# XiangFeng-Wen/STF-Unet

Hardware: AMD Instinct MI355X
Metric: training samples/sec (256x256 DCE-MRI frames) (higher is better)
Workload: dtype bf16; 1 GPU; cfg2 UNet(in=8,base_c=64) 256x256 train step; model=UNet, global_batch=64, per_gpu_batch=64, seq_len=8, parallelism=dp1, ddp_hook=False

## Files before the change

include/stfunet.h:

```cpp
#ifndef STFUNET_H
#define STFUNET_H
#include <stddef.h>
#include <stdint.h>

#ifdef __cplusplus
extern "C" {
#endif

typedef void* stf_stream_t;

typedef struct stf_conv_geom {
  int N;
  int Hs, Ws, Cs;
  int src_cstride;
  int Hd, Wd;
  int R, S;
  int stride, pad;
  int transposed;
} stf_conv_geom;

typedef struct stf_lstm_epi {
  const float* c_prev;
  float* c_out;
  void* h_out;
// ... 58 lines not shown

int stf_channel_sum(const void* x, int x_cstride, int M, int C, float* partial,
                    float* out, stf_stream_t stream);
int stf_stat_sums(const float* stats, int tiles, int Nout, int c0, int C, float* out, stf_stream_t stream);

int stf_bn_finalize(float* stats, int tiles, int groups, int C, int64_t M,
                    const float* gamma, const float* beta, float momentum, float eps,
                    float* running_mean, float* running_var, float* mean, float* invstd,
                    float* scale, float* shift, stf_stream_t stream);
typedef struct stf_bn_run_desc {
  const float* stats;
  float* running_mean;
  float* running_var;
  int64_t Mg;
  int tiles, groups, C;
  float momentum;
} stf_bn_run_desc;
int stf_bn_running_batch(const stf_bn_run_desc* descs, int count, stf_stream_t stream);
int stf_bn_act(const void* y, int y_cstride, int N, int H, int W, int C, int groups,
               const float* scale, const float* shift, int relu, const void* res,
               int res_cstride, const float* res_scale, const float* res_shift, void* out,
               int out_cstride, void* pooled, stf_stream_t stream);
int stf_bn_bwd_tiles(int N, int H, int W, int C, int groups, int pooled);
int stf_bn_bwd_reduce(const void* dz, int dz_cstride, const void* dpool, const void* y,
                      int y_cstride, int N, int H, int W, int C, int groups,
                      const float* scale, const float* shift, const float* mean,
                      const float* invstd, int mask_mode, const void* mask_src,
                      int mask_cstride, void* g_out, float* partial, stf_stream_t stream);
int stf_bn_bwd_finalize(float* partial, int tiles, int groups, int C, int64_t M,
                        const float* gamma, const float* mean, const float* invstd,
                        float* dgamma, float* dbeta, float* coef, stf_stream_t stream);
typedef struct stf_bn_gsum_desc {
  const float* partial;
  float* dgamma;
  float* dbeta;
  int tiles, groups, C;
} stf_bn_gsum_desc;
int stf_bn_groupsum_batch(const stf_bn_gsum_desc* descs, int count, stf_stream_t stream);
int stf_bn_bwd_apply_tiles(int64_t M, int C);
int stf_bn_bwd_apply(const void* g, int g_cstride, const void* y, int y_cstride, int64_t M,
                     int C, int groups, const float* mask_scale, const float* mask_shift,
                     const float* coef, void* dy, int dy_cstride, float* bias_partial,
                     float* dbias, stf_stream_t stream);

int stf_head_fwd(const void* y, int N, int H, int W, int C, const float* scale,
                 const float* shift, const float* w, const float* bias, int classes,
                 float* logits, stf_stream_t stream);
int stf_head_bwd(const float* dlogits, const void* y, int N, int H, int W, int C,
                 const float* scale, const float* shift, const float* mean,
                 const float* invstd, const float* w, int classes, void* g_out,
                 float* bn_partial, float* head_partial, float* dw, float* db,
                 stf_stream_t stream);
int stf_head_tiles(int N, int H, int W, int C);

int stf_loss_scratch_floats(int N, int classes);
int stf_loss_fwd(const float* logits, const int64_t* target, int N, int H, int W,
                 int classes, float* terms, float* loss, stf_stream_t stream);
int stf_loss_bwd(const float* logits, const int64_t* target, int N, int H, int W,
                 int classes, const float* terms, const float* grad_out, float* dlogits,
                 stf_stream_t stream);
int stf_loss_opt_scratch_floats(int N, int classes);
int stf_loss_opt_fwd(const float* logits, const int64_t* target, int N, int H, int W, int classes,
                     const float* class_weight, int ignore_index, int dice, float* terms,
                     float* loss, stf_stream_t stream);
int stf_loss_opt_bwd(const float* logits, const int64_t* target, int N, int H, int W, int classes,
                     const float* class_weight, int ignore_index, int dice, const float* terms,
                     const float* grad_out, float* dlogits, stf_stream_t stream);

int stf_adamw(float* p, const float* g, float* m, float* v, int64_t n, float lr,
              float beta1, float beta2, float eps, float weight_decay, float bc1,
              float bc2, stf_stream_t stream);
int stf_adamw_dev(float* p, const float* g, float* m, float* v, int64_t n, const float* hyper,
                  float beta1, float beta2, float eps, float weight_decay, stf_stream_t stream);
int stf_adamw_amp(float* p, const float* g, float* m, float* v, int64_t n, float* hyper,
                  const float* grad_scale, const float* found_inf, float beta1, float beta2, float eps,
                  float weight_decay, stf_stream_t stream);

int stf_pack_input(const float* x, int N, int C, int H, int W, int Cpad, void* out,
                   stf_stream_t stream);
int stf_pack_weight(const float* w, int d0, int d1, int R, int S, int mode, int cpad,
                    void* out, stf_stream_t stream);
typedef struct stf_pack_desc {
  const float* w;
  void* out;
  int d0, d1, R, S, mode, cpad;
} stf_pack_desc;
int stf_pack_weights(const stf_pack_desc* descs, int count, int64_t max_elems, stf_stream_t stream);
int stf_pack_tiles(int d0, int d1, int R, int S, int mode, int cpad);
int stf_pack_weights_tiled(const stf_pack_desc* descs, int count, int max_tiles, stf_stream_t stream);

int stf_pack_sequence(const float* x, int B, int Ttot, int C, int H, int W, int T, int P,
                      int Cpad, void* out, stf_stream_t stream);

int stf_stem_im2col(const float* x, int B, int Ttot, int C, int H, int W, int T, int P, int KS,
                    int stride, int pad, int Kpad, void* out, stf_stream_t stream);
int stf_stem_conv7_grid(int B, int T, int H, int W);
int stf_stem_conv7(const float* x, int B, int Ttot, int H, int W, int T, const void* w, void* y, float* stats,
                   stf_stream_t stream);
int stf_stem_wgrad7(const float* x, int B, int Ttot, int H, int W, int T, const void* dy, float* ws,
                    stf_stream_t stream);
int stf_stem_dgrad7(const void* dy, const float* w, int B, int Ttot, int Cf, int H, int W, int T, float* dx,
                    stf_stream_t stream);
int stf_maxpool3s2_fwd(const void* x, int N, int H, int W, int C, void* out, void* argmax,
                       stf_stream_t stream);
int stf_maxpool3s2_bwd(const void* argmax, const void* dout, int N, int H, int W, int C, void* dx,
                       stf_stream_t stream);
// ... 109 lines not shown
```

stf-unet_amd/csrc/common.h:

```cpp
#pragma once
#include <hip/hip_runtime.h>
#include <stdint.h>

#include <tuple>
#include <type_traits>
#include <utility>

#ifdef STF_FP16
typedef _Float16 e16;
#else
typedef __bf16 e16;
#endif
typedef e16 e16x8 __attribute__((ext_vector_type(8)));
typedef e16 e16x4 __attribute__((ext_vector_type(4)));
typedef short short4v __attribute__((ext_vector_type(4)));
typedef float f32x4 __attribute__((ext_vector_type(4)));
typedef float f32x16 __attribute__((ext_vector_type(16)));
typedef unsigned int u32x4v __attribute__((ext_vector_type(4)));

#define STF_DEV __device__ __forceinline__

STF_DEV float e2f(e16 v) { return (float)v; }
STF_DEV e16 f2e(float v) { return (e16)v; }

// ... 12 lines not shown
  return __uint_as_float(w << 16);
#endif
}
STF_DEV float hi16(uint32_t w) {
#ifdef STF_FP16
  return (float)__builtin_bit_cast(_Float16, (uint16_t)(w >> 16));
#else
  return __uint_as_float(w & 0xffff0000u);
#endif
}

STF_DEV void unpack8(const uint4& u, float (&f)[8]) {
  const uint32_t w[4] = {u.x, u.y, u.z, u.w};
#pragma unroll
  for (int i = 0; i < 4; ++i) {
    f[2 * i] = lo16(w[i]);
    f[2 * i + 1] = hi16(w[i]);
  }
}

STF_DEV uint32_t pack2(float a, float b) {
  e16 x = f2e(a), y = f2e(b);
  return (uint32_t)__builtin_bit_cast(uint16_t, x) | ((uint32_t)__builtin_bit_cast(uint16_t, y) << 16);
}

STF_DEV uint4 pack8(const float (&f)[8]) {
  return make_uint4(pack2(f[0], f[1]), pack2(f[2], f[3]), pack2(f[4], f[5]), pack2(f[6], f[7]));
}

STF_DEV float round_e(float v) { return e2f(f2e(v)); }

STF_DEV float sigm(float x) { return __builtin_amdgcn_rcpf(1.f + __expf(-x)); }
STF_DEV float tanh_f(float x) { return __builtin_fmaf(2.f, sigm(2.f * x), -1.f); }

STF_DEV void lstm_cell_fwd(float pi, float pf, float pg, float po, float cp, float& gi, float& gf, float& gg,
                           float& go, float& c, float& h) {
#pragma clang fp contract(off)
  gi = sigm(pi); gf = sigm(pf); gg = tanh_f(pg); go = sigm(po);
  c = __builtin_fmaf(gf, cp, gi * gg);
  h = go * tanh_f(c);
}
STF_DEV void lstm_cell_bwd(float gi, float gf, float gg, float go, float ct, float cp, float dh, float dcn,
                           float& d_i, float& d_f, float& d_g, float& d_o, float& dcp) {
#pragma clang fp contract(off)
  const float tc = tanh_f(ct);
  const float dct = __builtin_fmaf(dh * go, __builtin_fmaf(-tc, tc, 1.f), dcn);
  d_o = ((dh * tc) * go) * (1.f - go);
  d_i = ((dct * gg) * gi) * (1.f - gi);
  d_g = (dct * gi) * __builtin_fmaf(-gg, gg, 1.f);
  d_f = ((dct * cp) * gf) * (1.f - gf);
  dcp = dct * gf;
}

STF_DEV float wave_sum(float v) {
#pragma unroll
  for (int o = 32; o > 0; o >>= 1) v += __shfl_xor(v, o, 64);
  return v;
}

template <int CTRL>
STF_DEV float dpp_f(float v) {
  return __int_as_float(__builtin_amdgcn_update_dpp(0, __float_as_int(v), CTRL, 0xF, 0xF, true));
}

STF_DEV float row16_reduce_scatter(const float (&v)[16], int r) {
  float a[8], b[4], c[2];
  const bool h3 = r & 8, h2 = r & 4, h1 = r & 2, h0 = r & 1;
#pragma unroll
  for (int k = 0; k < 8; ++k) a[k] = (h3 ? v[k + 8] : v[k]) + dpp_f<0x140>(h3 ? v[k] : v[k + 8]);
#pragma unroll
  for (int k = 0; k < 4; ++k) b[k] = (h2 ? a[k + 4] : a[k]) + dpp_f<0x141>(h2 ? a[k] : a[k + 4]);
#pragma unroll
  for (int k = 0; k < 2; ++k) c[k] = (h1 ? b[k + 2] : b[k]) + dpp_f<0x1B>(h1 ? b[k] : b[k + 2]);
  return (h0 ? c[1] : c[0]) + dpp_f<0xB1>(h0 ? c[0] : c[1]);
}

STF_DEV double wave_sum_d(double v) {
#pragma unroll
  for (int o = 32; o > 0; o >>= 1) v += __shfl_xor(v, o, 64);
  return v;
}

namespace stf {
struct PlanOp {
  virtual ~PlanOp() {}
  virtual hipError_t run() const = 0;
};
bool plan_recording();
void plan_append(PlanOp* op, hipStream_t s);

template <class... A>
struct KernelOp final : PlanOp {
  const void* fn;
  dim3 grid, block;
  unsigned shmem;
  hipStream_t stream;
  std::tuple<A...> args;
  template <class... B>
  KernelOp(const void* f, dim3 g, dim3 b, unsigned sh, hipStream_t s, B&&... a)
      : fn(f), grid(g), block(b), shmem(sh), stream(s), args(std::forward<B>(a)...) {}
  hipError_t run() const override {
    return std::apply(
        [this](const A&... a) {
          void* p[sizeof...(A) + 1] = {const_cast<void*>(static_cast<const void*>(&a))...};
          return hipLaunchKernel(fn, grid, block, p, shmem, stream);
        },
// ... 36 lines not shown
```

stf-unet_amd/csrc/loss.hip:

```cpp
#include "common.h"
#include "../../include/stfunet.h"
#include "reduce.h"

namespace {

constexpr int NT = 256;
constexpr int MAXK = 4;
constexpr int LCHUNK = 64;
constexpr float DICE_EPS = 1e-6f;

STF_DEV void load8f(const float* p, float (&v)[8]) {
  const float4 a = *reinterpret_cast<const float4*>(p);
  const float4 b = *reinterpret_cast<const float4*>(p + 4);
  v[0] = a.x; v[1] = a.y; v[2] = a.z; v[3] = a.w; v[4] = b.x; v[5] = b.y; v[6] = b.z; v[7] = b.w;
}

STF_DEV float lane_group_sum(float v, int CG) {
  if (CG >= 2) v += dpp_f<0xB1>(v);
  if (CG >= 4) v += dpp_f<0x4E>(v);
  if (CG >= 8) v += dpp_f<0x141>(v);
  if (CG >= 16) v += dpp_f<0x140>(v);
  for (int o = 16; o < CG; o <<= 1) v += __shfl_xor(v, o, 64);
  return v;
}

int head_tiles(long units) {
  long t = (units + NT - 1) / NT;
  return (int)(t < 1 ? 1 : (t > 1024 ? 1024 : t));
}

template <int K>
__global__ void head_fwd_kernel(const uint16_t* __restrict__ y, long P, int HW, int C,
                                const float* __restrict__ scale, const float* __restrict__ shift,
                                const float* __restrict__ w, const float* __restrict__ bias,
                                float* __restrict__ logits) {
  constexpr int U = 4;
  const int CG = C / 8, cgs = __builtin_ctz(CG);
  const int units = (int)(P * CG);
  const int cg = (int)((blockIdx.x * NT + threadIdx.x) & (CG - 1));
  float sc[8], sh[8], wk[K][8], bk[K];
  load8f(scale + cg * 8, sc);
  load8f(shift + cg * 8, sh);
#pragma unroll
  for (int k = 0; k < K; ++k) { load8f(w + k * C + cg * 8, wk[k]); bk[k] = bias[k]; }
  const int stride = gridDim.x * NT;
  for (int u0 = blockIdx.x * NT; u0 < units; u0 += stride * U) {
    uint4 raw[U];
#pragma unroll
    for (int r = 0; r < U; ++r) {
      const int u = u0 + r * stride + threadIdx.x;
      raw[r] = u < units ? *reinterpret_cast<const uint4*>(y + (size_t)(u >> cgs) * C + cg * 8) : make_uint4(0, 0, 0, 0);
    }
#pragma unroll
    for (int r = 0; r < U; ++r) {
      const int u = u0 + r * stride + threadIdx.x;
      float v[8], acc[K];
      unpack8(raw[r], v);
#pragma unroll
      for (int k = 0; k < K; ++k) acc[k] = 0.f;
#pragma unroll
      for (int j = 0; j < 8; ++j) {
        const float a = fmaxf(v[j] * sc[j] + sh[j], 0.f);
#pragma unroll
        for (int k = 0; k < K; ++k) acc[k] += a * wk[k][j];
      }
#pragma unroll
      for (int k = 0; k < K; ++k) acc[k] = lane_group_sum(acc[k], CG);
      if (u < units && cg == 0) {
        const int pix = u >> cgs, n = pix / HW, hw = pix - n * HW;
#pragma unroll
        for (int k = 0; k < K; ++k) logits[(size_t)(n * K + k) * HW + hw] = acc[k] + bk[k];
      }
    }
  }
}

template <int K>
__global__ void head_bwd_kernel(const float* __restrict__ dlogits, const uint16_t* __restrict__ y, long P, int HW,
                                int C, const float* __restrict__ scale, const float* __restrict__ shift,
                                const float* __restrict__ mean, const float* __restrict__ invstd,
                                const float* __restrict__ w, uint16_t* __restrict__ g_out,
                                float* __restrict__ bn_partial, float* __restrict__ head_partial) {
  constexpr int NV = 16 + 8 * K + K;
  __shared__ float red[NT][NV + 1];
  const int CG = C / 8, cgs = __builtin_ctz(CG);
  const int units = (int)(P * CG);
  const int gt = blockIdx.x * NT + threadIdx.x;
  const int cg = gt & (CG - 1);
  float sc[8], sh[8], mu[8], is[8], wk[K][8];
  load8f(scale + cg * 8, sc);
  load8f(shift + cg * 8, sh);
  load8f(mean + cg * 8, mu);
  load8f(invstd + cg * 8, is);
#pragma unroll
  for (int k = 0; k < K; ++k) load8f(w + k * C + cg * 8, wk[k]);
  float sg[8] = {0, 0, 0, 0, 0, 0, 0, 0}, sgx[8] = {0, 0, 0, 0, 0, 0, 0, 0}, dw[K][8], db[K];
#pragma unroll
  for (int k = 0; k < K; ++k) {
    db[k] = 0.f;
#pragma unroll
    for (int j = 0; j < 8; ++j) dw[k][j] = 0.f;
  }
  constexpr int U = 1;
  const int S = gridDim.x * NT;
  for (int u0 = gt; u0 < units; u0 += S * U) {
    float dlr[U][K];
    uint4 yr[U];
    int pixr[U];
#pragma unroll
    for (int r = 0; r < U; ++r) {
      const int u = u0 + r * S;
      const bool ok = u < units;
      const int pix = ok ? u >> cgs : 0, n = pix / HW, hw = pix - n * HW;
      pixr[r] = ok ? pix : -1;
#pragma unroll
      for (int k = 0; k < K; ++k) dlr[r][k] = ok ? dlogits[(size_t)(n * K + k) * HW + hw] : 0.f;
      yr[r] = ok ? *reinterpret_cast<const uint4*>(y + (size_t)pix * C + cg * 8) : make_uint4(0, 0, 0, 0);
    }
#pragma unroll
    for (int r = 0; r < U; ++r) {
    if (pixr[r] < 0) continue;
    const int pix = pixr[r];
    const float* dl = dlr[r];
    float v[8], g[8];
    unpack8(yr[r], v);
#pragma unroll
    for (int j = 0; j < 8; ++j) {
      const float z = v[j] * sc[j] + sh[j];
      const float a = fmaxf(z, 0.f);
      float da = 0.f;
#pragma unroll
      for (int k = 0; k < K; ++k) { da += dl[k] * wk[k][j]; dw[k][j] += dl[k] * a; }
      g[j] = z > 0.f ? da : 0.f;
      sg[j] += g[j];
      sgx[j] += g[j] * (v[j] - mu[j]) * is[j];
    }
    if (cg == 0) {
#pragma unroll
      for (int k = 0; k < K; ++k) db[k] += dl[k];
    }
    *reinterpret_cast<uint4*>(g_out + (size_t)pix * C + cg * 8) = pack8(g);
    }
  }
#pragma unroll
  for (int j = 0; j < 8; ++j) { red[threadIdx.x][j] = sg[j]; red[threadIdx.x][8 + j] = sgx[j]; }
#pragma unroll
  for (int k = 0; k < K; ++k) {
#pragma unroll
    for (int j = 0; j < 8; ++j) red[threadIdx.x][16 + k * 8 + j] = dw[k][j];
    red[threadIdx.x][16 + 8 * K + k] = db[k];
  }
  __syncthreads();
  for (int c = threadIdx.x; c < C; c += NT) {
    const int gg = c / 8, j = c - gg * 8;
    float a = 0.f, b = 0.f;
    for (int t = gg; t < NT; t += CG) { a += red[t][j]; b += red[t][8 + j]; }
    bn_partial[(size_t)blockIdx.x * 2 * C + c] = a;
    bn_partial[(size_t)blockIdx.x * 2 * C + C + c] = b;
  }
  const int HC = K * (C + 1);
  for (int e = threadIdx.x; e < HC; e += NT) {
    float a = 0.f;
    if (e < K * C) {
      const int k = e / C, c = e - k * C, gg = c / 8, j = c - gg * 8;
      for (int t = gg; t < NT; t += CG) a += red[t][16 + k * 8 + j];
    } else {
      const int k = e - K * C;
      for (int t = 0; t < NT; t += CG) a += red[t][16 + 8 * K + k];
    }
    head_partial[(size_t)blockIdx.x * HC + e] = a;
  }
}

template <int K>
__global__ void loss_fwd_kernel(const float* __restrict__ logits, const int64_t* __restrict__ target, int HW,
                                float* __restrict__ part) {
  constexpr int NV = 3 * K + 1;
  __shared__ float red[NT / 64][NV];
  const int n = blockIdx.y;
  float s[NV];
#pragma unroll
  for (int i = 0; i < NV; ++i) s[i] = 0.f;
  for (int hw = blockIdx.x * NT + threadIdx.x; hw < HW; hw += gridDim.x * NT) {
    float z[K], e[K], mx = -INFINITY;
#pragma unroll
    for (int k = 0; k < K; ++k) { z[k] = logits[((long)n * K + k) * HW + hw]; mx = fmaxf(mx, z[k]); }
    float se = 0.f;
#pragma unroll
    for (int k = 0; k < K; ++k) { e[k] = expf(z[k] - mx); se += e[k]; }
    const int t = (int)target[(long)n * HW + hw];
    const float inv = 1.f / se, lse = logf(se);
#pragma unroll
    for (int k = 0; k < K; ++k) {
      const float p = e[k] * inv;
      const float tk = t == k ? 1.f : 0.f;
      s[3 * k] += p * tk;
      s[3 * k + 1] += p;
      s[3 * k + 2] += tk;
      if (t == k) s[3 * K] += lse - (z[k] - mx);
    }
  }
#pragma unroll
  for (int i = 0; i < NV; ++i) s[i] = wave_sum(s[i]);
  if ((threadIdx.x & 63) == 0)
#pragma unroll
    for (int i = 0; i < NV; ++i) red[threadIdx.x >> 6][i] = s[i];
  __syncthreads();
  if (threadIdx.x < NV) {
    float a = 0.f;
    for (int wv = 0; wv < NT / 64; ++wv) a += red[wv][threadIdx.x];
    part[((size_t)n * gridDim.x + blockIdx.x) * NV + threadIdx.x] = a;
  }
}

template <int K>
__global__ void loss_finalize_kernel(const float* __restrict__ part, int N, int HW, float* __restrict__ terms,
                                     float* __restrict__ loss) {
  constexpr int NV = 3 * K + 1;
  __shared__ double acc[64][NV];
  double ce = 0.0, dsum = 0.0;
  for (int base = 0; base < N; base += 64) {
    const int n = base + (int)threadIdx.x;
    if (threadIdx.x < 64) {
// ... 195 lines not shown
      }
      G[k] = dscale * dd;
      pg += p[k] * G[k];
    }
    const float cs = wt * inv_w;
#pragma unroll
    for (int k = 0; k < K; ++k) {
      const float tk = t == k ? 1.f : 0.f;
      const float g = go * ((p[k] - tk) * cs + p[k] * (G[k] - pg));
      dlogits[(n * K + k) * HW + hw] = keep ? g : 0.f;
    }
  }
}

__global__ void sum_tiles_kernel(const float* __restrict__ partial, int tiles, int C, int split,
                                 float* __restrict__ out, float* __restrict__ out2) {
  const int c = blockIdx.x * blockDim.x + threadIdx.x;
  if (c >= C) return;
  double s = 0.0;
  for (int t = 0; t < tiles; ++t) s += partial[(size_t)t * C + c];
  if (c < split) out[c] = (float)s;
  else out2[c - split] = (float)s;
}

bool head_ok(int C) { return C % 8 == 0 && C / 8 <= 64 && 64 % (C / 8) == 0; }

}

#define STF_KDISPATCH(K_, EXPR)             \
  switch (K_) {                             \
    case 1: { constexpr int KK = 1; EXPR; } break; \
    case 2: { constexpr int KK = 2; EXPR; } break; \
    case 3: { constexpr int KK = 3; EXPR; } break; \
    case 4: { constexpr int KK = 4; EXPR; } break; \
    default: return STF_EINVAL;             \
  }

extern "C" int stf_head_tiles(int N, int H, int W, int C) { return head_tiles((long)N * H * W * (C / 8)); }

extern "C" int stf_head_fwd(const void* y, int N, int H, int W, int C, const float* scale, const float* shift,
                            const float* w, const float* bias, int classes, float* logits, stf_stream_t stream) {
  if (!head_ok(C)) return STF_EINVAL;
  const long P = (long)N * H * W, units = P * (C / 8);
  if (units >= (1L << 31)) return STF_EINVAL;
  long blocks = (units + NT - 1) / NT;
  if (blocks > 8192) blocks = 8192;
  hipStream_t s = (hipStream_t)stream;
  STF_KDISPATCH(classes, hipLaunchKernelGGL(head_fwd_kernel<KK>, dim3(blocks), dim3(NT), 0, s, (const uint16_t*)y,
                                            P, H * W, C, scale, shift, w, bias, logits));
  STF_CHECK_LAUNCH();
  return 0;
}

extern "C" int stf_head_bwd(const float* dlogits, const void* y, int N, int H, int W, int C, const float* scale,
                            const float* shift, const float* mean, const float* invstd, const float* w, int classes,
                            void* g_out, float* bn_partial, float* head_partial, float* dw, float* db,
                            stf_stream_t stream) {
  if (!head_ok(C) || (long)N * H * W * (C / 8) >= (1L << 31)) return STF_EINVAL;
  const long P = (long)N * H * W;
  const int tiles = stf_head_tiles(N, H, W, C);
  hipStream_t s = (hipStream_t)stream;
  STF_KDISPATCH(classes, hipLaunchKernelGGL(head_bwd_kernel<KK>, dim3(tiles), dim3(NT), 0, s, dlogits,
                                            (const uint16_t*)y, P, H * W, C, scale, shift, mean, invstd, w,
                                            (uint16_t*)g_out, bn_partial, head_partial));
  STF_CHECK_LAUNCH();
  const int HC = classes * (C + 1);
  const int S = stf::colsum_stage1(head_partial, tiles, HC, s);
  hipLaunchKernelGGL(sum_tiles_kernel, dim3((HC + 255) / 256), dim3(256), 0, s, head_partial, S, HC, classes * C,
                     dw, db);
  STF_CHECK_LAUNCH();
  return 0;
}

extern "C" int stf_loss_scratch_floats(int N, int classes) {
  return N * classes * 3 + 1 + N * LCHUNK * (3 * classes + 1);
}

extern "C" int stf_loss_fwd(const float* logits, const int64_t* target, int N, int H, int W, int classes,
                            float* terms, float* loss, stf_stream_t stream) {
  hipStream_t s = (hipStream_t)stream;
  float* part = terms + N * classes * 3 + 1;
  STF_KDISPATCH(classes, {
    hipLaunchKernelGGL(loss_fwd_kernel<KK>, dim3(LCHUNK, N), dim3(NT), 0, s, logits, target, H * W, part);
    hipLaunchKernelGGL(loss_finalize_kernel<KK>, dim3(1), dim3(64), 0, s, part, N, H * W, terms, loss);
  });
  STF_CHECK_LAUNCH();
  return 0;
}

extern "C" int stf_loss_bwd(const float* logits, const int64_t* target, int N, int H, int W, int classes,
                            const float* terms, const float* grad_out, float* dlogits, stf_stream_t stream) {
  hipStream_t s = (hipStream_t)stream;
  const long P = (long)N * H * W;
  long blocks = (P + NT - 1) / NT;
  if (blocks > 8192) blocks = 8192;
  STF_KDISPATCH(classes, hipLaunchKernelGGL(loss_bwd_kernel<KK>, dim3(blocks), dim3(NT), 0, s, logits, target, N,
                                            H * W, terms, grad_out, dlogits));
  STF_CHECK_LAUNCH();
  return 0;
}

extern "C" int stf_loss_opt_scratch_floats(int N, int classes) {
  return N * classes * 3 + 2 + N * LCHUNK * (3 * classes + 2);
}

static bool loss_opt_ok(int classes, int ignore_index) {
  return classes >= 1 && classes <= MAXK && !(ignore_index >= 0 && ignore_index < classes);
}

extern "C" int stf_loss_opt_fwd(const float* logits, const int64_t* target, int N, int H, int W, int classes,
                                const float* class_weight, int ignore_index, int dice, float* terms, float* loss,
                                stf_stream_t stream) {
  if (!loss_opt_ok(classes, ignore_index)) return STF_EINVAL;
  hipStream_t s = (hipStream_t)stream;
  float* part = terms + N * classes * 3 + 2;
  STF_KDISPATCH(classes, {
    hipLaunchKernelGGL(loss_opt_fwd_kernel<KK>, dim3(LCHUNK, N), dim3(NT), 0, s, logits, target, H * W, class_weight,
                       ignore_index, part);
    hipLaunchKernelGGL(loss_opt_finalize_kernel<KK>, dim3(1), dim3(64), 0, s, part, N, dice, terms, loss);
  });
  STF_CHECK_LAUNCH();
  return 0;
// ... 16 lines not shown
```

stf-unet_amd/stfunet/_lib.py:

```python
import contextlib
import ctypes
import os

import torch

_HERE = os.path.dirname(os.path.abspath(__file__))
LIB_PATH = os.path.join(_HERE, "libstfunet_hip.so")
LIB_PATH = os.environ.get("STF_LIB", LIB_PATH)
LIB_PATH_F16 = os.environ.get("STF_LIB_F16", os.path.join(os.path.dirname(LIB_PATH), "libstfunet_hip_f16.so"))
LIB_PATHS = {torch.bfloat16: LIB_PATH, torch.float16: LIB_PATH_F16}
STORAGE_CODE = {torch.bfloat16: 0, torch.float16: 1}

BUILD_INFO = os.path.join(_HERE, "build_info.json")
_SRC_DIRS = (os.path.join(_HERE, "..", "csrc"), os.path.join(_HERE, "..", "..", "include"))


def _sha(paths):
    import hashlib
    h = hashlib.sha256()
    for p in paths:
        h.update(os.path.basename(p).encode())
        with open(p, "rb") as f:
            h.update(f.read())
    return h.hexdigest()[:16]
# ... 35 lines not shown
class ConvGeom(ctypes.Structure):
    _fields_ = [(n, c_int) for n in ("N", "Hs", "Ws", "Cs", "src_cstride", "Hd", "Wd", "R", "S",
                                     "stride", "pad", "transposed")]


class LstmEpi(ctypes.Structure):
    _fields_ = [("c_prev", P), ("c_out", P), ("h_out", P), ("h_cstride", c_int), ("gates", P),
                ("backward", c_int), ("dh", P), ("dh_cstride", c_int), ("dc_next", P), ("dc_prev", P),
                ("dgates", P)]


class BnrEpi(ctypes.Structure):
    _fields_ = [("y", P), ("y_cstride", c_int), ("scale", P), ("shift", P), ("mean", P), ("invstd", P),
                ("relu", c_int), ("partial", P)]


class IgemmArgs(ctypes.Structure):
    _fields_ = [("g", ConvGeom), ("src", P), ("wgt", P), ("Nout", c_int), ("dst", P),
                ("dst_cstride", c_int), ("bias", P), ("stats", P), ("scatter2x2", c_int),
                ("group_rows", c_int), ("accumulate", c_int), ("lstm", ctypes.POINTER(LstmEpi)),
                ("bnr", ctypes.POINTER(BnrEpi)), ("ws", P)]


class WgradArgs(ctypes.Structure):
    _fields_ = [("g", ConvGeom), ("dy", P), ("dy_cstride", c_int), ("Nout", c_int), ("x", P),
                ("ws", P), ("splits", c_int), ("grid_blocks", c_int)]


_SIGS = {
    "stf_igemm_stat_tiles": (c_int, [ctypes.POINTER(IgemmArgs)]),
    "stf_igemm_ws_bytes": (c_size_t, [ctypes.POINTER(IgemmArgs)]),
    "stf_igemm_bnr_tiles": (c_int, [ctypes.POINTER(IgemmArgs)]),
    "stf_igemm_kernel_name": (ctypes.c_char_p, [ctypes.POINTER(IgemmArgs)]),
    "stf_wgrad_kernel_name": (ctypes.c_char_p, [ctypes.POINTER(WgradArgs)]),
    "stf_igemm": (c_int, [ctypes.POINTER(IgemmArgs), P]),
    "stf_wgrad_plan": (c_int, [ctypes.POINTER(WgradArgs), ctypes.POINTER(c_int), ctypes.POINTER(c_size_t)]),
    "stf_wgrad": (c_int, [ctypes.POINTER(WgradArgs), P]),
    "stf_wgrad_reduce": (c_int, [P, c_int, c_int, c_int, c_int, c_int, P, P]),
    "stf_channel_sum": (c_int, [P, c_int, c_int, c_int, P, P, P]),
    "stf_bn_finalize": (c_int, [P, c_int, c_int, c_int, c_int64, P, P, c_float, c_float, P, P, P, P, P, P, P]),
    "stf_bn_running_batch": (c_int, [P, c_int, P]),
    "stf_bn_groupsum_batch": (c_int, [P, c_int, P]),
    "stf_bn_act": (c_int, [P, c_int, c_int, c_int, c_int, c_int, c_int, P, P, c_int, P, c_int, P, P, P, c_int, P,
                           P]),
    "stf_bn_bwd_tiles": (c_int, [c_int, c_int, c_int, c_int, c_int, c_int]),
    "stf_bn_bwd_reduce": (c_int, [P, c_int, P, P, c_int, c_int, c_int, c_int, c_int, c_int, P, P, P, P, c_int, P,
                                  c_int, P, P, P]),
    "stf_bn_bwd_finalize": (c_int, [P, c_int, c_int, c_int, c_int64, P, P, P, P, P, P, P]),
    "stf_bn_bwd_apply_tiles": (c_int, [c_int64, c_int]),
    "stf_bn_bwd_apply": (c_int, [P, c_int, P, c_int, c_int64, c_int, c_int, P, P, P, P, c_int, P, P, P]),
    "stf_head_fwd": (c_int, [P, c_int, c_int, c_int, c_int, P, P, P, P, c_int, P, P]),
    "stf_head_bwd": (c_int, [P, P, c_int, c_int, c_int, c_int, P, P, P, P, P, c_int, P, P, P, P, P, P]),
    "stf_head_tiles": (c_int, [c_int, c_int, c_int, c_int]),
    "stf_loss_scratch_floats": (c_int, [c_int, c_int]),
    "stf_loss_fwd": (c_int, [P, P, c_int, c_int, c_int, c_int, P, P, P]),
    "stf_loss_bwd": (c_int, [P, P, c_int, c_int, c_int, c_int, P, P, P, P]),
    "stf_loss_opt_scratch_floats": (c_int, [c_int, c_int]),
    "stf_loss_opt_fwd": (c_int, [P, P, c_int, c_int, c_int, c_int, P, c_int, c_int, P, P, P]),
    "stf_loss_opt_bwd": (c_int, [P, P, c_int, c_int, c_int, c_int, P, c_int, c_int, P, P, P, P]),
    "stf_adamw": (c_int, [P, P, P, P, c_int64, c_float, c_float, c_float, c_float, c_float, c_float, c_float,
                          P]),
    "stf_adamw_dev": (c_int, [P, P, P, P, c_int64, P, c_float, c_float, c_float, c_float, P]),
    "stf_adamw_amp": (c_int, [P, P, P, P, c_int64, P, P, P, c_float, c_float, c_float, c_float, P]),
    "stf_pack_input": (c_int, [P, c_int, c_int, c_int, c_int, c_int, P, P]),
    "stf_pack_weight": (c_int, [P, c_int, c_int, c_int, c_int, c_int, c_int, P, P]),
    "stf_pack_weights": (c_int, [P, c_int, c_int64, P]),
    "stf_augment_frames": (c_int, [P, P, c_int, P, P, c_int, c_int, c_float, c_float, P, P]),
    "stf_augment_masks": (c_int, [P, P, c_int, P, c_int, P, P]),
    "stf_pack_tiles": (c_int, [c_int, c_int, c_int, c_int, c_int, c_int]),
    "stf_pack_weights_tiled": (c_int, [P, c_int, c_int, P]),
    "stf_pack_sequence": (c_int, [P, c_int, c_int, c_int, c_int, c_int, c_int, c_int, c_int, P, P]),
    "stf_eval_counts": (c_int, [P, P, c_int, c_int, c_int64, c_int64, P, P, P]),
    "stf_lstm_coop_sync_bytes": (c_size_t, [c_int, c_int]),
    "stf_lstm_coop_supported": (c_int, [c_int]),
    "stf_lstm_coop_fwd": (c_int, [P, P, P, c_int, c_int, c_int, P, P, c_int, P, P, c_int, c_uint, P]),
    "stf_lstm_coop_bwd": (c_int, [P, P, P, c_int, c_int, c_int, P, c_int, P, P, c_int, P, c_int, c_uint, P]),
    "stf_lstm_coop_error": (c_int, [P, c_int, c_int, P, P]),
    "stf_bilinear_ac_fwd": (c_int, [P, c_int, c_int, c_int, c_int, c_int, P, c_int, c_int, c_int, P]),
    "stf_bilinear_ac_bwd": (c_int, [P, c_int, c_int, c_int, c_int, c_int, P, c_int, c_int, c_int, P]),
    "stf_stat_sums": (c_int, [P, c_int, c_int, c_int, c_int, P, P]),
    "stf_bilinear_ac_bwd_tsum": (c_int, [P, c_int, c_int, c_int, c_int, c_int, c_int, P, c_int64, c_int64, c_int,
                                         c_int, P]),
    "stf_eval_counts_sm": (c_int, [P, P, P, c_int, c_int, c_int64, c_int64, P, P, P]),
    "stf_predict_mask": (c_int, [P, P, c_int, c_int, c_int64, c_int, c_int, c_float, c_int64, P, P, P]),
    "stf_predict_overlay_scratch_bytes": (c_size_t, [c_int, c_int64]),
    "stf_predict_overlay": (c_int, [P, c_int64, P, c_int, c_int, c_int, c_int, c_int, c_int, c_float, c_int, P, P,
                                    P]),
    "stf_tofts_forward": (c_int, [P, P, P, c_int, c_int, P, P, P, P, P, c_int, c_float, P, P]),
    "stf_tofts_fit": (c_int, [P, c_int, c_int, P, P, P, P, P, c_int, c_float, c_int, c_int, P, c_float, c_float,
                              c_float, P, P, P]),
    "stf_stem_im2col": (c_int, [P, c_int, c_int, c_int, c_int, c_int, c_int, c_int, c_int, c_int, c_int, c_int, P,
                                P]),
    "stf_stem_conv7_grid": (c_int, [c_int, c_int, c_int, c_int]),
    "stf_stem_conv7": (c_int, [P, c_int, c_int, c_int, c_int, c_int, P, P, P, P]),
    "stf_stem_wgrad7": (c_int, [P, c_int, c_int, c_int, c_int, c_int, P, P, P]),
    "stf_stem_dgrad7": (c_int, [P, P, c_int, c_int, c_int, c_int, c_int, c_int, P, P]),
    "stf_maxpool3s2_fwd": (c_int, [P, c_int, c_int, c_int, c_int, P, P, P]),
    "stf_maxpool3s2_bwd": (c_int, [P, P, c_int, c_int, c_int, c_int, P, P]),
    "stf_bn_act_maxpool3s2": (c_int, [P, c_int, c_int, c_int, c_int, c_int, P, P, P, P, P]),
    "stf_bn_bwd_reduce_pool3": (c_int, [P, P, P, c_int, c_int, c_int, c_int, c_int, P, P, P, P, P, P]),
    "stf_bn_bwd_apply_pool3": (c_int, [P, P, P, c_int, c_int, c_int, c_int, c_int, P, P, P, P, P]),
    "stf_lstm_pack": (c_int, [P, P, P, P, c_int, P, P, P, P]),
    "stf_lstm_unpack_grad": (c_int, [P, P, c_int, P, P, P, P, P]),
    "stf_lstm_seq_fwd": (c_int, [P, P, P, c_int, c_int, c_int, P, P, c_int, P]),
    "stf_lstm_seq_supported": (c_int, [c_int]),
    "stf_lstm_seq_bwd": (c_int, [P, P, P, P, c_int, c_int, c_int, P, P, c_int, P, P, c_int, P]),
# ... 108 lines not shown
```

stf-unet_amd/stfunet/unet.py:

```python

import torch
import torch.nn as nn

from . import _lib, nhwc
from .flat import FlatParams
from .nhwc import Feat, new_feat
from .plan import StepRuntime


def _double_conv(cin, cout):
    return nn.Sequential(nn.Conv2d(cin, cout, 3, padding=1), nn.BatchNorm2d(cout), nn.ReLU(inplace=True),
                         nn.Conv2d(cout, cout, 3, padding=1), nn.BatchNorm2d(cout), nn.ReLU(inplace=True))


def _cpad(c):
    return (c + 7) // 8 * 8


class _Saved:
    pass


class DoubleConvProgram:

# ... 112 lines not shown
        dev = x.device
        S = _Saved()
        src = nhwc.pack_input(x, _cpad(m.in_channels))
        S.enc, S.cats = [], []
        h, w = H, W
        for lvl in self.levels:
            C = lvl.cout
            cat = new_feat(N, h, w, 2 * C, dev)
            pooled = new_feat(N, h // 2, w // 2, C, dev)
            S.enc.append(lvl.forward(src, training, need_bwd, out=cat.slice(C, C), pooled=pooled))
            S.cats.append(cat)
            src = pooled
            h, w = h // 2, w // 2
        Cb = self.bott.cout
        a_b = new_feat(N, h, w, Cb, dev)
        S.bott = self.bott.forward(src, training, need_bwd, out=a_b)
        cur = a_b
        S.dec, S.dec_in = [], []
        for i, (up, dec) in enumerate(zip(self.ups, self.decs)):
            cat = S.cats[3 - i]
            Clo = dec.cout
            wt = nhwc.pack_weight(up.weight, 2)
            nhwc.igemm(cur, wt, 4 * Clo, cat.slice(0, Clo), 1, 1, 1, 0, bias=up.bias.detach(), scatter2x2=True)
            S.dec_in.append(cur)
            last = i == 3
            if not last:
                out = new_feat(cat.N, cat.H, cat.W, Clo, dev)
                S.dec.append(dec.forward(cat, training, need_bwd, out=out))
                cur = out
            else:
                s = dec.forward(cat, training, True)
                S.dec.append(s)
        s = S.dec[-1]
        K = m.out_conv.out_channels
        logits = nhwc.empty((N, K, H, W), torch.float32, dev)
        S.head_w = m.out_conv.weight.detach().reshape(K, -1).contiguous()
        nhwc.call("stf_head_fwd", s.y2.ptr(), N, H, W, s.y2.C, nhwc._p(s.bn2.scale), nhwc._p(s.bn2.shift),
                  nhwc._p(S.head_w), nhwc._p(m.out_conv.bias.detach()), K, nhwc._p(logits), nhwc.stream())
        if not need_bwd:
            S.enc = S.cats = S.dec = None
        nhwc.flush_batches_tracked()
        return logits, (S if need_bwd else None)

    def _backward(self, S, dlogits):
        m = self.m
        gv = self.flat.grad_view
        dev = dlogits.device
        dlogits = dlogits.contiguous().float()
        s = S.dec[-1]
        N, K, H, W = dlogits.shape
        C = s.y2.C
        lib = nhwc._lib.load()
        tiles = lib.stf_head_tiles(N, H, W, C)
        g = new_feat(N, H, W, C, dev)
        bnp = nhwc.empty(tiles * 2 * C, torch.float32, dev)
        hp = nhwc.empty((tiles + 1) * K * (C + 1), torch.float32, dev)
        nhwc.call("stf_head_bwd", nhwc._p(dlogits), s.y2.ptr(), N, H, W, C, nhwc._p(s.bn2.scale),
                  nhwc._p(s.bn2.shift), nhwc._p(s.bn2.mean), nhwc._p(s.bn2.invstd), nhwc._p(S.head_w), K,
                  g.ptr(), nhwc._p(bnp), nhwc._p(hp), nhwc._p(gv(m.out_conv.weight)),
                  nhwc._p(gv(m.out_conv.bias)), nhwc.stream())
        dec1 = self.decs[3]
        dy2 = nhwc.bn_backward_from_partial(g, s.y2, s.bn2, dec1.blk[4], bnp, tiles, gv(dec1.blk[4].weight),
                                            gv(dec1.blk[4].bias), gv(dec1.blk[3].bias))
        dcat, cst, ctiles = dec1.backward(s, self.flat, True, dy2=dy2, dsrc_stats=True)
        self._done(dec1.blk)
        dcats = [None] * 4
        dcats[0] = (dcat, cst, ctiles)
        for i in (3, 2, 1, 0):
            up = self.ups[i]
            dcat, cst, ctiles = dcats[3 - i]
            dcats[3 - i] = dcat
            Clo = self.decs[i].cout
            dup = dcat.slice(0, Clo)
            src = S.dec_in[i]
            nhwc.wgrad(src, dup, 2, 2, 2, 0, gv(up.weight))
            nhwc.stat_sums(cst, ctiles, dcat.C, 0, Clo, gv(up.bias))
            dsrc = new_feat(src.N, src.H, src.W, src.C, dev)
            nhwc.igemm(dup, nhwc.pack_weight(up.weight, 3), src.C, dsrc, 2, 2, 2, 0)
            self._done(up)
            if i > 0:
                dcats[4 - i] = self.decs[i - 1].backward(S.dec[i - 1], self.flat, True, dz=dsrc, dsrc_stats=True)
                self._done(self.decs[i - 1].blk)
            else:
                d_b = dsrc
        dpool = self.bott.backward(S.bott, self.flat, True, dz=d_b)
        self._done(self.bott.blk)
        for j in (3, 2, 1, 0):
            lvl = self.levels[j]
            C = lvl.cout
            dskip = dcats[j].slice(C, C)
            dpool = lvl.backward(S.enc[j], self.flat, j > 0 or self.want_dx, dz=dskip, dpool=dpool)
            dcats[j] = None
            self._done(lvl.blk)
        if self.want_dx:
            self.dx = dpool.dense()[:, : m.in_channels].contiguous()


class _UNetFunction(torch.autograd.Function):
    @staticmethod
    def forward(ctx, x, prog, storage, res, *params):
        ctx.need_dx = ctx.needs_input_grad[0]
        if res is not None:
            logits, saved = res
            prog.runtime.own(saved, ctx)
        else:
            need_bwd = any(ctx.needs_input_grad[4:]) or ctx.need_dx
            with _lib.storage(storage):
                logits, saved = prog.forward(x, prog.m.training, need_bwd)
        ctx.storage = storage
        ctx.prog = prog
        ctx.saved = saved
        return logits.detach()

    @staticmethod
    def backward(ctx, dlogits):
        prog = ctx.prog
# ... 60 lines not shown
```

Baseline: 2747 samples/s.

## Recompute head gradient inside BN-backward apply instead of materializing it

Splits the head backward into a partials-only pass that skips writing the per-pixel gradient g, and a new apply kernel. The apply kernel recomputes g from dlogits, the head weights and the saved BN output, then applies the BN backward coefficients directly to produce dy2. This removes one full-resolution bf16 activation write and read at the top decoder level, at the cost of reloading y and dlogits and repeating the small K-class dot product. The eval-mode path keeps the old two-step route.

```diff
diff --git a/include/stfunet.h b/include/stfunet.h
--- a/include/stfunet.h
+++ b/include/stfunet.h
@@ -134,6 +134,14 @@
                  float* bn_partial, float* head_partial, float* dw, float* db,
                  stf_stream_t stream);
 int stf_head_tiles(int N, int H, int W, int C);
+int stf_head_bwd_partials(const float* dlogits, const void* y, int N, int H, int W, int C,
+                          const float* scale, const float* shift, const float* mean,
+                          const float* invstd, const float* w, int classes, float* bn_partial,
+                          float* head_partial, float* dw, float* db, stf_stream_t stream);
+int stf_head_bwd_apply(const float* dlogits, const float* w, int classes, const void* y,
+                       int y_cstride, int N, int H, int W, int C, const float* scale,
+                       const float* shift, const float* coef, void* dy, int dy_cstride,
+                       stf_stream_t stream);
 
 int stf_loss_scratch_floats(int N, int classes);
 int stf_loss_fwd(const float* logits, const int64_t* target, int N, int H, int W,
diff --git a/stf-unet_amd/csrc/common.h b/stf-unet_amd/csrc/common.h
--- a/stf-unet_amd/csrc/common.h
+++ b/stf-unet_amd/csrc/common.h
@@ -88,6 +88,20 @@
   dcp = dct * gf;
 }
 
+STF_DEV float bn_affine(float y, float sc, float sh) { return __builtin_fmaf(y, sc, sh); }
+STF_DEV float bn_bwd_dy(float A, float g, float B, float y, float C, int j) {
+#pragma clang fp contract(off)
+  const float ag = A * g, by = B * y;
+  return (j >= 6 ? ag + by : __builtin_fmaf(A, g, by)) + C;
+}
+template <int K>
+STF_DEV float head_da(const float (&dl)[K], const float (&wk)[K][8], int j) {
+  float da = 0.f;
+#pragma unroll
+  for (int k = 0; k < K; ++k) da = __builtin_fmaf(dl[k], wk[k][j], da);
+  return da;
+}
+
 STF_DEV float wave_sum(float v) {
 #pragma unroll
   for (int o = 32; o > 0; o >>= 1) v += __shfl_xor(v, o, 64);
diff --git a/stf-unet_amd/csrc/loss.hip b/stf-unet_amd/csrc/loss.hip
--- a/stf-unet_amd/csrc/loss.hip
+++ b/stf-unet_amd/csrc/loss.hip
@@ -76,7 +76,7 @@
 }
 
 template <int K>
-__global__ void head_bwd_kernel(const float* __restrict__ dlogits, const uint16_t* __restrict__ y, long P, int HW,
+__global__ __launch_bounds__(K > 2 ? NT : 1024) void head_bwd_kernel(const float* __restrict__ dlogits, const uint16_t* __restrict__ y, long P, int HW,
                                 int C, const float* __restrict__ scale, const float* __restrict__ shift,
                                 const float* __restrict__ mean, const float* __restrict__ invstd,
                                 const float* __restrict__ w, uint16_t* __restrict__ g_out,
@@ -121,16 +121,16 @@
     for (int r = 0; r < U; ++r) {
     if (pixr[r] < 0) continue;
     const int pix = pixr[r];
-    const float* dl = dlr[r];
+    const float (&dl)[K] = dlr[r];
     float v[8], g[8];
     unpack8(yr[r], v);
 #pragma unroll
     for (int j = 0; j < 8; ++j) {
-      const float z = v[j] * sc[j] + sh[j];
+      const float z = bn_affine(v[j], sc[j], sh[j]);
       const float a = fmaxf(z, 0.f);
-      float da = 0.f;
-#pragma unroll
-      for (int k = 0; k < K; ++k) { da += dl[k] * wk[k][j]; dw[k][j] += dl[k] * a; }
+      const float da = head_da<K>(dl, wk, j);
+#pragma unroll
+      for (int k = 0; k < K; ++k) dw[k][j] += dl[k] * a;
       g[j] = z > 0.f ? da : 0.f;
       sg[j] += g[j];
       sgx[j] += g[j] * (v[j] - mu[j]) * is[j];
@@ -139,7 +139,7 @@
 #pragma unroll
       for (int k = 0; k < K; ++k) db[k] += dl[k];
     }
-    *reinterpret_cast<uint4*>(g_out + (size_t)pix * C + cg * 8) = pack8(g);
+    if (g_out) *reinterpret_cast<uint4*>(g_out + (size_t)pix * C + cg * 8) = pack8(g);
     }
   }
 #pragma unroll
@@ -169,6 +169,56 @@
       for (int t = 0; t < NT; t += CG) a += red[t][16 + 8 * K + k];
     }
     head_partial[(size_t)blockIdx.x * HC + e] = a;
+  }
+}
+
+constexpr int HUPT = 4;
+template <int K>
+__global__ __launch_bounds__(NT) void head_bwd_apply_kernel(const float* __restrict__ dlogits,
+                                                            const uint16_t* __restrict__ y, int ycs, int P, int HW,
+                                                            int cgs, const float* __restrict__ scale,
+                                                            const float* __restrict__ shift,
+                                                            const float* __restrict__ w,
+                                                            const float* __restrict__ coef,
+                                                            uint16_t* __restrict__ dy, int dycs) {
+  const int CG = 1 << cgs, C = 8 << cgs;
+  const int units = P << cgs, S = gridDim.x * NT * HUPT;
+  const int cg = threadIdx.x & (CG - 1);
+  float A[8], B[8], Cc[8], sc[8], sh[8], wk[K][8];
+  load8f(coef + cg * 8, A);
+  load8f(coef + C + cg * 8, B);
+  load8f(coef + 2 * C + cg * 8, Cc);
+  load8f(scale + cg * 8, sc);
+  load8f(shift + cg * 8, sh);
+#pragma unroll
+  for (int k = 0; k < K; ++k) load8f(w + k * C + cg * 8, wk[k]);
+  for (int u = blockIdx.x * NT * HUPT + threadIdx.x; u < units; u += S) {
+    uint4 yq[HUPT];
+    float dlr[HUPT][K];
+#pragma unroll
+    for (int r = 0; r < HUPT; ++r) {
+      const int ur = u + r * NT;
+      if (ur < units) {
+        const int pix = ur >> cgs, n = pix / HW, hw = pix - n * HW;
+#pragma unroll
+        for (int k = 0; k < K; ++k) dlr[r][k] = dlogits[(size_t)(n * K + k) * HW + hw];
+        yq[r] = *reinterpret_cast<const uint4*>(y + (size_t)pix * ycs + cg * 8);
+      }
+    }
+#pragma unroll
+    for (int r = 0; r < HUPT; ++r) {
+      const int ur = u + r * NT;
+      if (ur >= units) break;
+      float v[8];
+      unpack8(yq[r], v);
+#pragma unroll
+      for (int j = 0; j < 8; ++j) {
+        const float z = bn_affine(v[j], sc[j], sh[j]);
+        const float g = round_e(z > 0.f ? head_da<K>(dlr[r], wk, j) : 0.f);
+        v[j] = bn_bwd_dy(A[j], g, B[j], v[j], Cc[j], j);
+      }
+      *reinterpret_cast<uint4*>(dy + (size_t)(ur >> cgs) * dycs + cg * 8) = pack8(v);
+    }
   }
 }
 
@@ -470,10 +520,10 @@
   return 0;
 }
 
-extern "C" int stf_head_bwd(const float* dlogits, const void* y, int N, int H, int W, int C, const float* scale,
-                            const float* shift, const float* mean, const float* invstd, const float* w, int classes,
-                            void* g_out, float* bn_partial, float* head_partial, float* dw, float* db,
-                            stf_stream_t stream) {
+static int head_bwd(const float* dlogits, const void* y, int N, int H, int W, int C, const float* scale,
+                    const float* shift, const float* mean, const float* invstd, const float* w, int classes,
+                    void* g_out, float* bn_partial, float* head_partial, float* dw, float* db,
+                    stf_stream_t stream) {
   if (!head_ok(C) || (long)N * H * W * (C / 8) >= (1L << 31)) return STF_EINVAL;
   const long P = (long)N * H * W;
   const int tiles = stf_head_tiles(N, H, W, C);
@@ -486,6 +536,41 @@
   const int S = stf::colsum_stage1(head_partial, tiles, HC, s);
   hipLaunchKernelGGL(sum_tiles_kernel, dim3((HC + 255) / 256), dim3(256), 0, s, head_partial, S, HC, classes * C,
                      dw, db);
+  STF_CHECK_LAUNCH();
+  return 0;
+}
+
+extern "C" int stf_head_bwd(const float* dlogits, const void* y, int N, int H, int W, int C, const float* scale,
+                            const float* shift, const float* mean, const float* invstd, const float* w, int classes,
+                            void* g_out, float* bn_partial, float* head_partial, float* dw, float* db,
+                            stf_stream_t stream) {
+  if (!g_out) return STF_EINVAL;
+  return head_bwd(dlogits, y, N, H, W, C, scale, shift, mean, invstd, w, classes, g_out, bn_partial, head_partial,
+                  dw, db, stream);
+}
+
+extern "C" int stf_head_bwd_partials(const float* dlogits, const void* y, int N, int H, int W, int C,
+                                     const float* scale, const float* shift, const float* mean,
+                                     const float* invstd, const float* w, int classes, float* bn_partial,
+                                     float* head_partial, float* dw, float* db, stf_stream_t stream) {
+  return head_bwd(dlogits, y, N, H, W, C, scale, shift, mean, invstd, w, classes, nullptr, bn_partial,
+                  head_partial, dw, db, stream);
+}
+
+extern "C" int stf_head_bwd_apply(const float* dlogits, const float* w, int classes, const void* y, int y_cstride,
+                                  int N, int H, int W, int C, const float* scale, const float* shift,
+                                  const float* coef, void* dy, int dy_cstride, stf_stream_t stream) {
+  if (!dlogits || !w || !y || !scale || !shift || !coef || !dy) return STF_EINVAL;
+  if (!head_ok(C) || y_cstride % 8 || dy_cstride % 8 || y_cstride < C || dy_cstride < C) return STF_EINVAL;
+  if ((((uintptr_t)y | (uintptr_t)dy) & 15) || N < 1 || H < 1 || W < 1) return STF_EINVAL;
+  const long P = (long)N * H * W, units = P * (C / 8);
+  long blocks = (units + (long)NT * HUPT - 1) / ((long)NT * HUPT);
+  if (blocks > 8192) blocks = 8192;
+  if (units + blocks * NT * HUPT >= (1L << 31)) return STF_EINVAL;
+  STF_KDISPATCH(classes, hipLaunchKernelGGL(head_bwd_apply_kernel<KK>, dim3(blocks), dim3(NT), 0,
+                                            (hipStream_t)stream, dlogits, (const uint16_t*)y, y_cstride, (int)P,
+                                            H * W, __builtin_ctz(C / 8), scale, shift, w, coef, (uint16_t*)dy,
+                                            dy_cstride));
   STF_CHECK_LAUNCH();
   return 0;
 }
diff --git a/stf-unet_amd/stfunet/_lib.py b/stf-unet_amd/stfunet/_lib.py
--- a/stf-unet_amd/stfunet/_lib.py
+++ b/stf-unet_amd/stfunet/_lib.py
@@ -111,6 +111,8 @@
     "stf_head_fwd": (c_int, [P, c_int, c_int, c_int, c_int, P, P, P, P, c_int, P, P]),
     "stf_head_bwd": (c_int, [P, P, c_int, c_int, c_int, c_int, P, P, P, P, P, c_int, P, P, P, P, P, P]),
     "stf_head_tiles": (c_int, [c_int, c_int, c_int, c_int]),
+    "stf_head_bwd_partials": (c_int, [P, P, c_int, c_int, c_int, c_int, P, P, P, P, P, c_int, P, P, P, P, P]),
+    "stf_head_bwd_apply": (c_int, [P, P, c_int, P, c_int, c_int, c_int, c_int, c_int, P, P, P, P, c_int, P]),
     "stf_loss_scratch_floats": (c_int, [c_int, c_int]),
     "stf_loss_fwd": (c_int, [P, P, c_int, c_int, c_int, c_int, P, P, P]),
     "stf_loss_bwd": (c_int, [P, P, c_int, c_int, c_int, c_int, P, P, P, P]),
diff --git a/stf-unet_amd/stfunet/unet.py b/stf-unet_amd/stfunet/unet.py
--- a/stf-unet_amd/stfunet/unet.py
+++ b/stf-unet_amd/stfunet/unet.py
@@ -188,16 +188,28 @@
         C = s.y2.C
         lib = nhwc._lib.load()
         tiles = lib.stf_head_tiles(N, H, W, C)
-        g = new_feat(N, H, W, C, dev)
         bnp = nhwc.empty(tiles * 2 * C, torch.float32, dev)
         hp = nhwc.empty((tiles + 1) * K * (C + 1), torch.float32, dev)
-        nhwc.call("stf_head_bwd", nhwc._p(dlogits), s.y2.ptr(), N, H, W, C, nhwc._p(s.bn2.scale),
-                  nhwc._p(s.bn2.shift), nhwc._p(s.bn2.mean), nhwc._p(s.bn2.invstd), nhwc._p(S.head_w), K,
-                  g.ptr(), nhwc._p(bnp), nhwc._p(hp), nhwc._p(gv(m.out_conv.weight)),
-                  nhwc._p(gv(m.out_conv.bias)), nhwc.stream())
         dec1 = self.decs[3]
-        dy2 = nhwc.bn_backward_from_partial(g, s.y2, s.bn2, dec1.blk[4], bnp, tiles, gv(dec1.blk[4].weight),
-                                            gv(dec1.blk[4].bias), gv(dec1.blk[3].bias))
+        bn2 = dec1.blk[4]
+        if s.bn2.training:
+            nhwc.call("stf_head_bwd_partials", nhwc._p(dlogits), s.y2.ptr(), N, H, W, C, nhwc._p(s.bn2.scale),
+                      nhwc._p(s.bn2.shift), nhwc._p(s.bn2.mean), nhwc._p(s.bn2.invstd), nhwc._p(S.head_w), K,
+                      nhwc._p(bnp), nhwc._p(hp), nhwc._p(gv(m.out_conv.weight)), nhwc._p(gv(m.out_conv.bias)),
+                      nhwc.stream())
+            coef = nhwc._bn_bwd_coef(s.y2, s.bn2, bn2, bnp, tiles, gv(bn2.weight), gv(bn2.bias))
+            dy2 = new_feat(N, H, W, C, dev)
+            nhwc.call("stf_head_bwd_apply", nhwc._p(dlogits), nhwc._p(S.head_w), K, s.y2.ptr(), s.y2.cs, N, H, W,
+                      C, nhwc._p(s.bn2.scale), nhwc._p(s.bn2.shift), nhwc._p(coef), dy2.ptr(), dy2.cs,
+                      nhwc.stream())
+        else:
+            g = new_feat(N, H, W, C, dev)
+            nhwc.call("stf_head_bwd", nhwc._p(dlogits), s.y2.ptr(), N, H, W, C, nhwc._p(s.bn2.scale),
+                      nhwc._p(s.bn2.shift), nhwc._p(s.bn2.mean), nhwc._p(s.bn2.invstd), nhwc._p(S.head_w), K,
+                      g.ptr(), nhwc._p(bnp), nhwc._p(hp), nhwc._p(gv(m.out_conv.weight)),
+                      nhwc._p(gv(m.out_conv.bias)), nhwc.stream())
+            dy2 = nhwc.bn_backward_from_partial(g, s.y2, s.bn2, bn2, bnp, tiles, gv(bn2.weight), gv(bn2.bias),
+                                                gv(dec1.blk[3].bias))
         dcat, cst, ctiles = dec1.backward(s, self.flat, True, dy2=dy2, dsrc_stats=True)
         self._done(dec1.blk)
         dcats = [None] * 4
```

Measured after the change: 2768 samples/s, median of 6. No clear change (+0.8%).
